# HiKapok/X-Detector

Measured on AMD Instinct MI355X. Metric: images/sec at 480x480 Light-Head R-CNN, 1/2/4/8 MI355X + backbone MFMA util%, higher is better.
Workload: dtype f16x3 (split-precision f16 MFMA, f32 accumulate, f32 activations); 1 GPU; Full Light-Head R-CNN (Xception backbone + RPN + GPU proposals/NMS + PSROIAlign + light head + per-class NMS), 300 proposals, 480x480; batch_per_gpu=256, global_batch=256, image_size=480, concurrent_sub_batches=2, cross_terms=f16, input=whitened f32 [B,3,480,480] resident in HBM, parallelism=image-sharded dp1, weights=seeded random init (no checkpoint exists), graph_replay=True

## Files before the change

include/xdet.h:

```cpp
#ifndef XDET_H_
#define XDET_H_

#include <stddef.h>
#include <stdint.h>

#ifdef __cplusplus
extern "C" {
#endif

#define XDET_OK 0
#define XDET_ERR_INVALID_ARG (-1)
#define XDET_ERR_HIP (-2)
#define XDET_ERR_STATE (-3)
#define XDET_ERR_UNSUPPORTED (-4)

const char* xdet_last_error(void);
int xdet_version(void);
int xdet_device_count(int* n);
int xdet_set_device(int dev);
int xdet_device_pci_bus_id(int dev, char* buf, int buflen);
int xdet_probe_ipc(void);
int xdet_set_default_precision(int mode);
int xdet_get_default_precision(void);

// ... 65 lines not shown
size_t xdet_spectral_conv_workspace_bytes(void* layer, int N);
int xdet_spectral_conv_forward(void* layer, const float* in, int N, int ld_in, void* workspace, float* out, int ld_out,
                               void* stream);
int xdet_stem_conv3x3s2_forward(const float* in_nchw, const float* w27x32, const float* scale, const float* shift,
                                uint16_t* out_hi, uint16_t* out_lo, int N, int S, void* stream);
int xdet_resnet_stem7x7_forward(void* layer, const float* in_nchw, int N, int S, float* out, void* stream);
int xdet_maxpool3x3s2_bn_planes(const float* in, const float* scale, const float* shift, uint16_t* out_hi, uint16_t* out_lo,
                                int N, int H, int W, int C, int ld, float mul, uint16_t* out_hi2, uint16_t* out_lo2,
                                int c32_2, float mul2, void* stream);
int xdet_resnet_preconv_forward(void* layer, const float* pre_scale, const float* pre_shift, const float* x, int N, int H,
                                int W, uint16_t* out_hi, uint16_t* out_lo, void* stream);
int xdet_sepconv_fused_hpool_forward(void* dw_layer, void* pw_layer, const float* in, int N, int H, int W, int ld_in,
                                     float* out_hpooled, int ld_out, int relu_in, void* stream);
int xdet_maxpool_v3s2_add(const float* in_hpooled, const float* residual, float* out, int N, int H, int Wo, int C, int ld,
                          void* stream);
int xdet_maxpool3x3s2_add(const float* in, const float* residual, float* out, int N, int H, int W, int C, int ld,
                          void* stream);
int xdet_nchw_to_nhwc4(const float* in_nchw, float* out_nhwc4, int N, int C, int H, int W, void* stream);
int xdet_preprocess_eval(const uint8_t* image_hwc, int H, int W, float* out_chw, int out_size, void* stream);
enum { XDET_RESIZE_NONE = 1, XDET_RESIZE_CENTRAL_CROP = 2, XDET_RESIZE_PAD_AND_RESIZE = 3, XDET_RESIZE_WARP = 4 };
int xdet_preprocess_eval_batch(const uint8_t* packed, int64_t packed_bytes, const int64_t* offsets,
                               const int32_t* image_shapes, int N, int out_size, int resize, float* out_nchw,
                               float* bbox_img, void* stream);
size_t xdet_preprocess_train_workspace_bytes(int N, int G);
int xdet_preprocess_train_batch(const uint8_t* packed, int64_t packed_bytes, const int64_t* offsets,
                                const int32_t* image_shapes, const int32_t* glabels, const float* gbboxes,
                                const int32_t* n_gt, const int32_t* image_ids , int N, int G,
                                int out_size, uint32_t seed, float* out_nchw, int32_t* out_glabels, float* out_gbboxes,
                                int32_t* out_n_gt, void* records , void* workspace, void* stream);

// ... 173 lines not shown
```

x-detector_amd/csrc/cabi.hip:

```cpp
#include "lighthead.h"
#include "resnet_trunk.h"

namespace xdet {

static thread_local std::string g_last_error;
void set_last_error(const std::string& s) { g_last_error = s; }
int hip_fail(hipError_t e, const char* what, const char* file, int line) {
  char buf[512];
  snprintf(buf, sizeof(buf), "HIP error %d (%s) at %s:%d: %s", (int)e, hipGetErrorString(e), file, line, what);
  g_last_error = buf;
  return XDET_ERR_HIP;
}

static inline hipStream_t S(void* s) { return reinterpret_cast<hipStream_t>(s); }

int g_default_precision = PREC_F32;

}

using namespace xdet;

extern "C" {

const char* xdet_last_error(void) { return g_last_error.c_str(); }
// ... 357 lines not shown
  XDET_REQUIRE(D->ld == ld_in && L->ld_in() == ld_in && L->ld_out() == ld_out && ld_out <= L->cout_pad &&
                   sepconv_fused_supported(ld_in, L->cout_pad, D->dil),
               "sepconv_fused: needs <= 256 input channels (multiple of 32), <= 128 or 129..1024 outputs, dilation 1");
  int Wo, pl;
  same_pad(W, 3, 2, 1, &pl, &Wo);
  DeviceGuard guard(L->device);
  return launch_sepconv_fused(in, D->d_w, L->d_wt_hi_b, L->d_wt_lo_b, L->d_scale, L->d_shift, out_hpooled, N, H, W, ld_in,
                              ld_out, L->cout_pad, relu_in, L->relu_out, S(stream), pl);
}
int xdet_maxpool_v3s2_add(const float* in_hpooled, const float* residual, float* out, int N, int H, int Wo, int C, int ld,
                          void* stream) {
  int Ho, pt;
  same_pad(H, 3, 2, 1, &pt, &Ho);
  return launch_maxpool_v3s2_add(in_hpooled, residual, out, N, H, Wo, C, ld, Ho, pt, S(stream));
}
int xdet_maxpool3x3s2_add(const float* in, const float* residual, float* out, int N, int H, int W, int C, int ld,
                          void* stream) {
  int Ho, Wo, pt, pl;
  same_pad(H, 3, 2, 1, &pt, &Ho);
  same_pad(W, 3, 2, 1, &pl, &Wo);
  return launch_maxpool3x3s2_add(in, residual, out, N, H, W, C, ld, Ho, Wo, pt, pl, S(stream));
}
int xdet_preprocess_eval(const uint8_t* image_hwc, int H, int W, float* out_chw, int out_size, void* stream) {
  return launch_preprocess_eval(image_hwc, H, W, out_chw, out_size, S(stream));
}
int xdet_preprocess_eval_batch(const uint8_t* packed, int64_t packed_bytes, const int64_t* offsets,
                               const int32_t* image_shapes, int N, int out_size, int resize, float* out_nchw,
                               float* bbox_img, void* stream) {
  return launch_preprocess_batch(packed, packed_bytes, offsets, image_shapes, N, out_size, resize, out_nchw, bbox_img,
                                 S(stream));
// ... 101 lines not shown
  XDET_REQUIRE(!n->built, "set_option: the net is already built");
  const std::string k(key), v(value);
  if (k == "large_sep") {
    XDET_REQUIRE(v == "auto" || v == "direct" || v == "spectral", "large_sep must be auto | direct | spectral");
    n->large_sep_mode = v == "auto" ? 0 : v == "direct" ? 1 : 2;
    return XDET_OK;
  }
  if (k == "rpn_stream") {
    XDET_REQUIRE(v == "side" || v == "main", "rpn_stream must be side | main");
    n->rpn_side_stream = v == "side";
    return XDET_OK;
  }
  if (k == "pool_sub") {
    XDET_REQUIRE(v == "on" || v == "off", "pool_sub: on | off");
    n->pool_writes_projection_input = v == "on";
    return XDET_OK;
  }
  if (k == "workspace") {
    XDET_REQUIRE(v == "reuse" || v == "ssa" || v == "poison", "workspace: reuse | ssa | poison");
    XDET_REQUIRE(!(v != "ssa" && n->check_range), "workspace=reuse: check_range validates every tensor after the forward and needs workspace=ssa");
    n->reuse_workspace = v != "ssa";
    n->poison_recycled = v == "poison";
    return XDET_OK;
  }
  if (k == "sepconv") {
    XDET_REQUIRE(v == "fused" || v == "split", "sepconv must be fused | split");
    n->fuse_sepconv = v == "fused";
    return XDET_OK;
  }
  if (k == "ksplit") {
// ... 366 lines not shown
```

x-detector_amd/csrc/common.h:

```cpp
#pragma once
#include <hip/hip_runtime.h>
#include "../../include/xdet.h"
#include "conv_params.h"
#include "workspace.h"
#include <atomic>
#include <cstdint>
#include <cstdio>
#include <string>
#include <vector>

namespace xdet {

void set_last_error(const std::string& s);
int hip_fail(hipError_t e, const char* what, const char* file, int line);

#define XDET_HIP(expr)                                                          \
  do {                                                                          \
    hipError_t _e = (expr);                                                     \
    if (_e != hipSuccess) return ::xdet::hip_fail(_e, #expr, __FILE__, __LINE__); \
  } while (0)

#define XDET_LAUNCH_CHECK() XDET_HIP(hipGetLastError())

#define XDET_REQUIRE(cond, msg)                                   \
// ... 78 lines not shown
                   unsigned short* lo, hipStream_t s);
int launch_dft_inv(const float* Y, int F, int ldn, int C_ld, int N, int m_pad, const float* tab, const float* scale,
                   const float* shift, int relu, float* out, int ldo, int axis, hipStream_t s);

bool sepconv_fused_supported(int cin_ld, int cout_pad, int dil);
int launch_sepconv_fused(const float* in, const float* w9c, const unsigned short* wt_hi_blocked,
                         const unsigned short* wt_lo_blocked, const float* scale, const float* shift, float* out, int N,
                         int H, int W, int ld, int ldo, int cout_pad, int relu_in, int relu_out, hipStream_t s,
                         int pool_pad_l = -1);

bool conv3x3_patch_supported(int kh, int kw, int cin, int cout_pad, int stride, int dil, int pad_mode);
int launch_conv3x3_patch(const unsigned short* in_hi, const unsigned short* in_lo, const unsigned short* wt_hi_blocked,
                         const unsigned short* wt_lo_blocked, const float* scale, const float* shift, float* out, int N, int H,
                         int W, int ldo, int relu, hipStream_t s);

bool resnet_stem7x7_supported(int kh, int kw, int cin, int cout, int stride, int pad_mode, int pad, int S);
int launch_resnet_stem7x7(const float* img_nchw, const unsigned short* wt_hi, const unsigned short* wt_lo, const float* scale,
                          const float* shift, float* out, int N, int S, hipStream_t s);

bool resnet_preconv_supported(int cin, int cmid, int64_t M);
int launch_resnet_preconv(const float* x, const float* pre_sc, const float* pre_sh, const unsigned short* w_hi,
                          const unsigned short* w_lo, const float* sc, const float* sh, unsigned short* out_hi,
                          unsigned short* out_lo, int64_t M, int cin, int cmid, hipStream_t s);

struct BneckLaunch {
  const float* x;
  const float *pre_sc, *pre_sh;
  const unsigned short *wa_hi, *wa_lo, *wb_hi, *wb_lo, *wc_hi, *wc_lo;
  const float *sc_a, *sh_a, *sc_b, *sh_b, *sc_c, *sh_c;
  const float *pl_sc, *pl_sh;
// ... 73 lines not shown
```

x-detector_amd/csrc/lighthead.hip:

```cpp
#include "lighthead.h"

namespace xdet {

static inline double nsplit_of(const ConvLayer* L) { return L->precision == PREC_F16X3 ? 3.0 : 1.0; }

int LightHeadNet::build_body() {
  const float eps = 1e-4f;
  const int S = cfg.image_size;
  in4.H = S; in4.W = S; in4.C = 3;
  XDET_TRY(new_buf(S, S, 3, &in4));
  Buf x, r, t;
  if (g_default_precision != PREC_F32) {
    const HostTensor* kt;
    XDET_TRY(need("block1_conv1/kernel", &kt, {3, 3, 3, 32}));
    std::vector<float> sc, sh;
    float *d_w, *d_sc, *d_sh;
    XDET_TRY(upload(kt->v, &d_w));
    XDET_TRY(upload_bn("block1_conv1_bn", 32, 32, eps, &sc, &sh, &d_sc, &d_sh));
    x = Buf();
    x.H = x.W = (S - 3) / 2 + 1; x.C = 32; x.ld = 32; x.no_f32 = true;
    XDET_TRY(new_planes(&x));
    pscales[x.pidx].name = "block1_conv1 [stem]";
    const Pow2Scaled bn_sc{sc, d_sc}, bn_sh{sh, d_sh};
    pscales[x.pidx].apply.push_back([=](int e) {
// ... 15 lines not shown
  c2.k = 3; c2.cout = 64; c2.pad_mode = 0; c2.relu_out = 1;
  XDET_TRY(conv_bn("block1_conv2", "block1_conv2_bn", eps, ST_BODY, x, c2, &t));
  XDET_REQUIRE(!keep_stem_out || (t.p && !t.no_f32), "plan: stem_out=keep, but block1_conv2 writes no f32 output");
  x = t;
  struct Blk { const char* res; const char* bn; const char* s1; const char* s2; int c; int first_relu; };
  const Blk blks[3] = {{"conv2d_1", "batch_normalization_1", "block2_sepconv1", "block2_sepconv2", 128, 0},
                       {"conv2d_2", "batch_normalization_2", "block3_sepconv1", "block3_sepconv2", 256, 1},
                       {"conv2d_3", "batch_normalization_3", "block4_sepconv1", "block4_sepconv2", 728, 1}};
  Buf presub;
  bool x_is_relu = false;
  for (int bi = 0; bi < 3; ++bi) {
    const Blk& b = blks[bi];
    ConvArgs proj;
    proj.cout = b.c; proj.stride = 2;
    if (presub.hi) proj.presub = &presub;
    XDET_TRY(conv_bn(b.res, b.bn, eps, ST_BODY, x, proj, &r));
    Buf a, p;
    SepArgs s1;
    s1.cout = b.c; s1.pre_relu = x_is_relu ? 0 : b.first_relu; s1.relu_out = 1;
    XDET_TRY(sep_bn(b.s1, eps, ST_BODY, x, s1, &a));
    Buf nsub;
    const bool two_readers = bi < 2 && pool_writes_projection_input && subsample_projections &&
                             g_default_precision != PREC_F32 && b.c % 32 == 0;
    SepArgs s2;
    s2.cout = b.c; s2.pool_res = &r;
    if (two_readers) s2.next_sub = &nsub;
    XDET_TRY(sep_bn(b.s2, eps, ST_BODY, a, s2, &p));
    presub = nsub;
    x_is_relu = nsub.hi != nullptr;
    if (bi == 0 && keep_stem_out) stem_out = x;
    else release_f32(x);
    release_f32(a);
    release_f32(r);
    x = p;
  }
  for (int blk = 5; blk <= 12; ++blk) {
    const Buf res = x;
    Buf a, b2, c3;
    const std::string pre = "block" + std::to_string(blk);
    SepArgs sep;
// ... 325 lines not shown
```

x-detector_amd/csrc/plan.h:

```cpp
#pragma once
#include "layers.h"

#include <array>
#include <functional>
#include <map>
#include <memory>

namespace xdet {

struct HostTensor {
  std::vector<float> v;
  std::vector<int64_t> dims;
};
typedef std::map<std::string, HostTensor> WeightMap;

struct Buf {
  float* p = nullptr;
  unsigned short *hi = nullptr, *lo = nullptr;
  bool planes_relu = false;
  bool no_f32 = false;
  int pidx = -1;
  int H = 0, W = 0, C = 0, ld = 0;
  size_t per_image() const { return (size_t)H * W * ld; }
};

struct ConvEmit {
  int planes = 0;
  const Buf* into = nullptr;
  const std::vector<float>* bn_scale = nullptr;
  const std::vector<float>* bn_shift = nullptr;
  int* optional = nullptr;
  bool ksplit = false;
};

struct ConvArgs {
  int k = 1, cout = 0, stride = 1;
  int pad_mode = 1;
  int pad_expl = 0;
  int relu_out = 0, relu_in = 0;
  const Buf* res = nullptr;
  const float *pre_sc = nullptr, *pre_sh = nullptr;
  const Buf* presub = nullptr;
  ConvEmit emit;
};

struct SepArgs {
  int cout = 0, pre_relu = 0, dilation = 1, relu_out = 0;
  const Buf* res = nullptr;
  const Buf* pool_res = nullptr;
  Buf* next_sub = nullptr;
  ConvEmit emit;
};

struct GraphCache {
  typedef std::array<uintptr_t, 10> Key;
  static constexpr size_t kMax = 8;
  std::map<Key, hipGraphExec_t> execs;
  std::vector<Key> order;
  void clear() {
    for (auto& g : execs) (void)hipGraphExecDestroy(g.second);
    execs.clear();
    order.clear();
  }
  int launch(const Key& key, hipStream_t s, const std::function<int()>& forward) {
    auto it = execs.find(key);
// ... 167 lines not shown

  std::vector<char> planes_drop_ok;
  virtual bool planes_dropped() const { return false; }
  int ksplit_design_batch = 0;
  bool ksplit_all = false;
  static int pow2_floor(int64_t v) { int r = 1; while ((int64_t)r * 2 <= v) r *= 2; return r; }
  int maybe_ksplit(ConvLayer* L, int Hi, int Wi, int Ho, int Wo, bool marked);
  struct KsLayer { ConvLayer* L; bool aux; };
  std::vector<KsLayer> ks_layers;
  float* ks_slab[2] = {nullptr, nullptr};
  int* ks_ticket[2] = {nullptr, nullptr};
  int finish_ksplit();
  bool fuse_sepconv = true;
  bool subsample_projections = true;
  bool pool_writes_projection_input = true;
  bool patch_conv3x3 = true;
  bool fuse_hpool = true;
  int pool_fuse_min_pixels = 100 * 100;
  int add_conv(const std::string& name, int stage, const Buf& in_, ConvLayer* L, const Buf* res, int relu_in, Buf* out,
               const ConvEmit& em = {});
  int add_dw(const std::string& name, int stage, const Buf& in, DepthwiseLayer* L, int relu_in, Buf* out,
             bool planes_only = false);
  int add_pool(const std::string& name, int stage, const Buf& in, const Buf* res, Buf* out);
  ConvLayer* keep(ConvLayer* L) { layers.emplace_back(L); return L; }
  DepthwiseLayer* keep(DepthwiseLayer* L) { layers.emplace_back(L); return L; }
  SpectralConv* keep(SpectralConv* L) { layers.emplace_back(L); return L; }

  int conv_bn(const std::string& name, const std::string& bn, float eps, int stage, const Buf& in, const ConvArgs& args, Buf* out,
              ConvLayer** layer = nullptr);
  int sep_bn(const std::string& name, float eps, int stage, const Buf& in, const SepArgs& args, Buf* out);
// ... 6 lines not shown
```

x-detector_amd/csrc/plan.hip:

```cpp
#include "plan.h"

#include <cstdlib>

namespace xdet {

int Plan::take(size_t bytes, void** out, int kind, size_t slack_bytes) {
  bytes = std::max<size_t>(bytes, 256);
  if (reuse_workspace) {
    auto& fl = ws_free[ws_pool][kind];
    auto it = kind == 1 ? fl.find(bytes) : fl.lower_bound(bytes);
    if (it != fl.end() && it->first <= 2 * bytes) {
      *out = it->second;
      const size_t block = it->first;
      fl.erase(it);
      ws_bytes[*out] = block;
      ws_recycled_bytes += bytes;
      if (poison_recycled && kind == 0 && bytes > slack_bytes)
        poison.push_back({ops.size(), reinterpret_cast<float*>(static_cast<char*>(*out) + (bytes - slack_bytes)),
                          (block - (bytes - slack_bytes)) / 4});
      return XDET_OK;
    }
  }
  XDET_TRY(alloc_bytes(bytes, out));
  ws_bytes[*out] = bytes;
// ... 322 lines not shown
  std::vector<float> sc, sh;
  const float *scp = nullptr, *shp = nullptr;
  if (!bn.empty()) {
    XDET_TRY(fold_bn(bn, cout, eps, nullptr, &sc, &sh));
    scp = sc.data(); shp = sh.data();
  }
  ConvLayer* L = keep(new ConvLayer());
  if (layer) *layer = L;
  XDET_REQUIRE(!pre_sc || (k == 1 && stride == 2 && g_default_precision != PREC_F32 && in.C >= 32 && !in.no_f32 &&
                           in.ld % 32 == 0),
               "plan: a pre-activation can only be folded into a 1x1 stride-2 projection on the split path");
  if (k == 1 && stride == 2 && (pad_mode == 1 || (pad_mode == 2 && pad_expl == 0)) &&
      g_default_precision != PREC_F32 && in.C >= 32 && in.ld % 32 == 0 && !relu_in && !in.no_f32 &&
      (subsample_projections || pre_sc)) {
    XDET_TRY(L->init(1, 1, in.C, cout, 1, 1, 1, 0, 0, kt->v.data(), scp, shp, relu_out));
    if (presub && presub->hi) {
      XDET_REQUIRE(!pre_sc && presub->H == (in.H + 1) / 2 && presub->W == (in.W + 1) / 2 && presub->ld == in.ld,
                   "plan: pre-made subsampled planes do not match the projection's input");
      XDET_TRY(add_conv(name, stage, *presub, L, res, 0, out, emit));
      release_planes(*presub);
      return XDET_OK;
    }
    Buf sub;
    sub.H = (in.H + 1) / 2; sub.W = (in.W + 1) / 2; sub.C = in.C; sub.ld = in.ld; sub.no_f32 = true;
    XDET_TRY(new_planes(&sub));
    pscales[sub.pidx].name = name + "/subsample_split";
    const Buf i = in, o = sub;
    ops.push_back({name + "/subsample_split", stage, 0.0, [=](int N, hipStream_t s) {
                     return launch_split_f32_subsample2(i.p, o.hi, o.lo, N, i.H, i.W, i.ld, s, pre_sc, pre_sh, pmul(o.pidx));
                   }});
    XDET_TRY(add_conv(name, stage, sub, L, res, 0, out, emit));
    release_planes(sub);
    return XDET_OK;
  }
  XDET_REQUIRE(!(presub && presub->hi), "plan: pre-made subsampled planes, but this conv is not a subsampled 1x1 / stride-2 projection");
  XDET_TRY(L->init(k, k, in.C, cout, stride, 1, pad_mode, pad_expl, pad_expl, kt->v.data(), scp, shp, relu_out));
  if (patch_conv3x3 && L->dma_capable() && in.hi && !in.planes_relu && !relu_in && !res && emit.planes == 0 &&
      in.ld == 32 && conv3x3_patch_supported(k, k, in.C, L->cout_pad, stride, 1, pad_mode) && L->cout_pad == L->ld_out()) {
    XDET_TRY(new_buf(in.H - 2, in.W - 2, cout, out));
    if (in.pidx >= 0) pscales[in.pidx].apply.push_back([L](int e) { return L->set_in_exp(e); });
    const Buf i = in, o = *out;
    ops.push_back({name + " [LDS-staged tile]", stage, L->flops(in.H, in.W), [=](int N, hipStream_t s) {
                     return launch_conv3x3_patch(i.hi, i.lo, L->d_wt_hi_b, L->d_wt_lo_b, L->d_scale, L->d_shift, o.p, N, i.H,
                                                 i.W, o.ld, L->relu_out, s);
                   }});
// ... 4 lines not shown

int Plan::sep_bn(const std::string& name, float eps, int stage, const Buf& in, const SepArgs& args, Buf* out) {
  const int cout = args.cout, pre_relu = args.pre_relu, dilation = args.dilation, relu_out = args.relu_out;
  const Buf *res = args.res, *pool_res = args.pool_res;
  Buf* next_sub = args.next_sub;
  const ConvEmit& emit = args.emit;
  const HostTensor *dk, *pk;
  XDET_TRY(need(name + "/depthwise_kernel", &dk, {3, 3, in.C, 1}));
  XDET_TRY(need(name + "/pointwise_kernel", &pk, {1, 1, in.C, cout}));
  DepthwiseLayer* D = keep(new DepthwiseLayer());
  XDET_TRY(D->init(in.C, dilation, dk->v.data()));
  std::vector<float> sc, sh;
  XDET_TRY(fold_bn(name + "_bn", cout, eps, nullptr, &sc, &sh));
  ConvLayer* L = keep(new ConvLayer());
  XDET_TRY(L->init(1, 1, in.C, cout, 1, 1, 1, 0, 0, pk->v.data(), sc.data(), sh.data(), relu_out));
  if (fuse_sepconv && L->dma_capable() && !res && emit.planes == 0 && !in.no_f32 &&
      sepconv_fused_supported(in.ld, L->cout_pad, dilation) && L->ld_out() <= L->cout_pad) {
    {
      PlaneScale ps;
      ps.name = name + " (depthwise result inside the fused block)";
      ps.src = in.p;
      ps.src_per_image = in.per_image();
      ps.src_relu = pre_relu;
      float bound = 0.f;
      for (int c = 0; c < in.C; ++c) {
        float a = 0.f;
        for (int t = 0; t < 9; ++t) a += std::fabs(dk->v[(size_t)t * in.C + c]);
        bound = std::max(bound, a);
      }
      ps.bound = bound;
      ps.apply.push_back([D](int e) { return D->set_out_exp(e); });
      ps.apply.push_back([L](int e) { return L->set_in_exp(e); });
      ps.op_index = (int)ops.size();
      pscales.push_back(ps);
    }
    if (pool_res && fuse_hpool && in.H * in.W >= pool_fuse_min_pixels) {
      int Ho, Wo, pt, pl;
      same_pad(in.H, 3, 2, 1, &pt, &Ho);
      same_pad(in.W, 3, 2, 1, &pl, &Wo);
      Buf hp;
      XDET_TRY(new_buf(in.H, Wo, cout, &hp));
      XDET_TRY(new_buf(Ho, Wo, cout, out));
      XDET_REQUIRE(pool_res->H == Ho && pool_res->W == Wo && pool_res->ld == out->ld && !pool_res->no_f32,
                   "plan: pool residual shape mismatch");
      const Buf i = in, h = hp, o = *out;
      const float* rp = pool_res->p;
      ops.push_back({name + "/fused_dw+pw+hpool", stage, L->flops(in.H, in.W), [=](int N, hipStream_t s) {
                       return launch_sepconv_fused(i.p, D->d_w, L->d_wt_hi_b, L->d_wt_lo_b, L->d_scale, L->d_shift, h.p, N,
                                                   i.H, i.W, i.ld, h.ld, L->cout_pad, pre_relu, L->relu_out, s, pl);
                     }});
      Buf sub;
      if (next_sub && out->ld % 32 == 0) {
        sub.H = (Ho + 1) / 2; sub.W = (Wo + 1) / 2; sub.C = out->C; sub.ld = out->ld; sub.no_f32 = true;
        XDET_TRY(new_planes(&sub));
        pscales[sub.pidx].name = name + "/vpool_add (subsampled planes for the next projection)";
        *next_sub = sub;
      }
      const Buf sb = sub;
      ops.push_back({name + (sb.hi ? "/vpool_add+subsample_split+relu" : "/vpool_add"), stage, 0.0, [=](int N, hipStream_t s) {
                       return launch_maxpool_v3s2_add(h.p, rp, o.p, N, h.H, h.W, h.C, h.ld, Ho, pt, s, sb.hi, sb.lo,
                                                      sb.hi ? pmul(sb.pidx) : 1.f);
                     }});
      release_f32(hp);
      return XDET_OK;
    }
    Buf full;
    Buf* dst = pool_res ? &full : out;
    XDET_TRY(new_buf(in.H, in.W, cout, dst));
    const Buf i = in, o = *dst;
    ops.push_back({name + "/fused_dw+pw", stage, L->flops(in.H, in.W), [=](int N, hipStream_t s) {
                     return launch_sepconv_fused(i.p, D->d_w, L->d_wt_hi_b, L->d_wt_lo_b, L->d_scale, L->d_shift, o.p, N,
                                                 i.H, i.W, i.ld, o.ld, L->cout_pad, pre_relu, L->relu_out, s);
                   }});
    if (!pool_res) return XDET_OK;
    XDET_TRY(add_pool(name + "/pool_add", stage, full, pool_res, out));
    release_f32(full);
    return XDET_OK;
  }
  Buf t, full;
  XDET_TRY(add_dw(name + "/depthwise", stage, in, D, pre_relu, &t, L->dma_capable()));
  XDET_TRY(add_conv(name + "/pointwise", stage, t, L, res, 0, pool_res ? &full : out, emit));
  release_planes(t);
  release_f32(t);
  if (!pool_res) return XDET_OK;
  XDET_TRY(add_pool(name + "/pool_add", stage, full, pool_res, out));
  release_f32(full);
  return XDET_OK;
}

int Plan::run_stage(int stage, int N, hipStream_t s) {
  for (size_t i = 0; i < ops.size(); ++i) {
    const Op& op = ops[i];
    if (op.stage != stage) continue;
    for (const PoisonRec& pr : poison)
      if (pr.op == i) XDET_HIP(hipMemsetD32Async(reinterpret_cast<hipDeviceptr_t>(pr.at), 0x7fc00000, pr.words, s));
    if (profiling) {
      ProfRec r;
      r.op = (int)i;
      XDET_HIP(hipEventCreate(&r.a));
      XDET_HIP(hipEventCreate(&r.b));
      XDET_HIP(hipEventRecord(r.a, s));
// ... 41 lines not shown
```

x-detector_amd/xdet/_lib.py:

```python
import ctypes
import os

_HERE = os.path.dirname(os.path.abspath(__file__))
LIB_PATH = os.environ.get('XDET_LIB') or os.path.join(_HERE, 'libxdet_hip.so')

c_void_p = ctypes.c_void_p
c_int = ctypes.c_int
c_float = ctypes.c_float
c_size_t = ctypes.c_size_t
c_int64 = ctypes.c_int64
c_double = ctypes.c_double
PF = c_void_p
PI = c_void_p


class XdetError(RuntimeError):
    def __init__(self, code, msg):
        RuntimeError.__init__(self, 'xdet error %d: %s' % (code, msg))
        self.code = code


class InvalidArgumentError(XdetError, ValueError):
    """XDET_ERR_INVALID_ARG: the counterpart of tf.errors.InvalidArgumentError raised by the
    reference op's OP_REQUIRES checks (cpp/PSROIPooling/ps_roi_align_op.cc:209-226)."""
# ... 62 lines not shown
    'xdet_sepconv_fused_forward': (c_int, [c_void_p, c_void_p, PF, c_int, c_int, c_int, c_int, PF, c_int, c_int, c_void_p]),
    'xdet_conv3x3_patch_forward': (c_int, [c_void_p, c_void_p, c_void_p, c_int, c_int, c_int, PF, c_int, c_void_p]),
    'xdet_resnet_bneck_forward': (c_int, [c_void_p, c_void_p, c_void_p, PF, PF, PF, c_int, c_int, c_int, PF, PF, PF,
                                          c_void_p, c_void_p, c_void_p]),
    'xdet_spectral_conv_create': (c_int, [ctypes.POINTER(c_void_p), PF, c_int, c_int, c_int, c_int, c_int, PF, PF, c_int]),
    'xdet_spectral_conv_workspace_bytes': (c_size_t, [c_void_p, c_int]),
    'xdet_spectral_conv_forward': (c_int, [c_void_p, PF, c_int, c_int, c_void_p, PF, c_int, c_void_p]),
    'xdet_stem_conv3x3s2_forward': (c_int, [PF, PF, PF, PF, c_void_p, c_void_p, c_int, c_int, c_void_p]),
    'xdet_resnet_stem7x7_forward': (c_int, [c_void_p, PF, c_int, c_int, PF, c_void_p]),
    'xdet_maxpool3x3s2_bn_planes': (c_int, [PF, PF, PF, c_void_p, c_void_p, c_int, c_int, c_int, c_int, c_int, c_float,
                                            c_void_p, c_void_p, c_int, c_float, c_void_p]),
    'xdet_resnet_preconv_forward': (c_int, [c_void_p, PF, PF, PF, c_int, c_int, c_int, c_void_p, c_void_p, c_void_p]),
    'xdet_sepconv_fused_hpool_forward': (c_int, [c_void_p, c_void_p, PF, c_int, c_int, c_int, c_int, PF, c_int, c_int,
                                                 c_void_p]),
    'xdet_maxpool_v3s2_add': (c_int, [PF, PF, PF, c_int, c_int, c_int, c_int, c_int, c_void_p]),
    'xdet_maxpool3x3s2_add': (c_int, [PF, PF, PF, c_int, c_int, c_int, c_int, c_int, c_void_p]),
    'xdet_preprocess_eval': (c_int, [c_void_p, c_int, c_int, PF, c_int, c_void_p]),
    'xdet_preprocess_eval_batch': (c_int, [c_void_p, c_int64, c_void_p, PI, c_int, c_int, c_int, PF, PF, c_void_p]),
    'xdet_preprocess_train_workspace_bytes': (c_size_t, [c_int, c_int]),
    'xdet_preprocess_train_batch': (c_int, [c_void_p, c_int64, c_void_p, PI, PI, PF, PI, PI, c_int, c_int, c_int, ctypes.c_uint32,
                                            PF, PI, PF, PI, c_void_p, c_void_p, c_void_p]),
    'xdet_nchw_to_nhwc4': (c_int, [PF, PF, c_int, c_int, c_int, c_int, c_void_p]),
    'xdet_rpn_decode': (c_int, [PF, c_int, c_int, c_int, c_int, c_int, c_int, c_int, PF, PF, PF, PF, c_void_p]),
    'xdet_proposals_workspace_bytes': (c_size_t, [c_int, c_int, c_int, c_int]),
    'xdet_get_proposals': (c_int, [PF, PF, c_int, c_int, c_int, c_int, c_float, c_float, c_void_p, PF, PI, c_void_p]),
    'xdet_ext_decode_rois': (c_int, [PF, PF, c_int, c_int64, PF, c_void_p]),
    'xdet_bboxes_eval': (c_int, [PF, c_int, PF, c_int, c_int, c_int, PI, PF, c_int, c_int, c_float, c_float, c_int,
                                 PF, PF, c_void_p]),
    'xdet_head_decode_probs': (c_int, [PF, PF, c_int, c_int, c_int, c_int64, c_int, PF, PF, PI, c_void_p]),
    'xdet_bboxes_eval_probs': (c_int, [PF, PF, c_int, c_int, c_int, PI, PF, c_int, c_int, c_float, c_float, c_int, PI,
# ... 130 lines not shown
```

x-detector_amd/xdet/build.py:

```python
import os
import subprocess
import sys

HERE = os.path.dirname(os.path.abspath(__file__))
CSRC = os.path.join(os.path.dirname(HERE), 'csrc')
LIB = os.path.join(HERE, 'libxdet_hip.so')

SOURCES = [
    ('conv_mfma.hip', []),
    ('conv_mfma_split.hip', []),
    ('conv_mfma_dma.hip', []),
    ('conv_mfma_ksplit.hip', []),
    ('elementwise.hip', []),
    ('spectral.hip', []),
    ('sepconv_fused.hip', []),
    ('conv3x3_patch.hip', []),
    ('resnet_bneck.hip', []),
    ('resnet_stem.hip', []),
    ('resnet_preconv.hip', []),
    ('psroialign.hip', ['-ffp-contract=off']),
    ('psroialign_grad_ordered.hip', ['-ffp-contract=off']),
    ('rotated_psroialign.hip', ['-ffp-contract=off']),
    ('proposals.hip', ['-ffp-contract=off']),
    ('detect.hip', ['-ffp-contract=off']),
    ('evalmatch.hip', ['-ffp-contract=off']),
    ('targets.hip', ['-ffp-contract=off']),
    ('losses.hip', ['-ffp-contract=off']),
    ('dense_backward.hip', []),
    ('conv_backward.hip', []),
    ('batchnorm.hip', ['-ffp-contract=off']),
    ('depthwise_backward.hip', ['-ffp-contract=off']),
# ... 48 lines not shown
```

x-detector_amd/xdet/model.py:

```python
import contextlib
import ctypes

import numpy as np

from ._lib import lib, check, c_void_p, LightHeadConfig, XdetError, InvalidArgumentError
from .runtime import DeviceBuffer, DeviceTensor, Stream, to_host, synchronize, _host, _current, _det, _sync
from . import train as _train
from .train import *


class LightHeadDetector(object):
    def __init__(self, weights, image_size=480, max_batch=1, num_classes=21, rpn_pre_nms_top_n=5000,
                 rpn_post_nms_top_n=1000, rpn_nms_thres=0.7, rpn_min_size=None, select_threshold=0.01,
                 nms_threshold=0.3, nms_topk=200, device=None, large_sep='auto', sepconv='fused', rpn_stream='side',
                 conv3x3='patch', pool='split', check_range=False, ksplit=True, cross='f16', workspace=None, pool_sub=None,
                 pool_index=False, rpn_hidden=False, large_sep_train=False, exit_flow_train=False, middle_flow_train=False,
                 entry_flow_train=False):
        stages = (large_sep_train, exit_flow_train, middle_flow_train, entry_flow_train)
        _train.check_stages(stages, weights)
        if device is not None:
            check(lib().xdet_set_device(int(device)))
        self.cfg = LightHeadConfig(image_size=image_size, max_batch=max_batch, num_classes=num_classes,
                                   rpn_pre_nms_top_n=rpn_pre_nms_top_n, rpn_post_nms_top_n=rpn_post_nms_top_n,
                                   rpn_nms_thres=rpn_nms_thres,
                                   rpn_min_size=(16. / 480) if rpn_min_size is None else rpn_min_size,
                                   select_threshold=select_threshold, nms_threshold=nms_threshold, nms_topk=nms_topk)
        h = c_void_p()
        check(lib().xdet_net_create(ctypes.byref(h), ctypes.byref(self.cfg)))
        self.handle = h
        self._head_kernels = {}
        self._rpn_kernels = {}
# ... 3 lines not shown
                self._head_kernels[name] = a
            if rpn_hidden and name in ('rpn_head/conv2d/kernel', 'rpn_head/conv2d_1/kernel', 'rpn_head/conv2d_2/kernel'):
                self._rpn_kernels[name] = a
            dims = (ctypes.c_int64 * a.ndim)(*a.shape)
            check(lib().xdet_net_set_weight(self.handle, name.encode(), _host(a), a.ndim, dims))
        check(lib().xdet_net_set_option(self.handle, b'large_sep', large_sep.encode()))
        check(lib().xdet_net_set_option(self.handle, b'sepconv', sepconv.encode()))
        check(lib().xdet_net_set_option(self.handle, b'rpn_stream', rpn_stream.encode()))
        check(lib().xdet_net_set_option(self.handle, b'conv3x3', conv3x3.encode()))
        check(lib().xdet_net_set_option(self.handle, b'pool', pool.encode()))
        check(lib().xdet_net_set_option(self.handle, b'check_range', b'on' if check_range else b'off'))
        if workspace is not None:
            check(lib().xdet_net_set_option(self.handle, b'workspace', workspace.encode()))
        if pool_sub is not None:
            check(lib().xdet_net_set_option(self.handle, b'pool_sub', pool_sub.encode()))
        check(lib().xdet_net_set_option(self.handle, b'ksplit', ksplit.encode() if isinstance(ksplit, str) else (b'on' if ksplit else b'off')))
        check(lib().xdet_net_set_option(self.handle, b'cross', cross.encode()))
        if pool_index:
            check(lib().xdet_net_set_option(self.handle, b'pool_index', b'keep'))
        if rpn_hidden:
            check(lib().xdet_net_set_option(self.handle, b'rpn_hidden', b'keep'))
        if middle_flow_train:
            check(lib().xdet_net_set_option(self.handle, b'entry_x', b'keep'))
        if entry_flow_train:
            check(lib().xdet_net_set_option(self.handle, b'stem_out', b'keep'))
        self.pool_index, self.rpn_hidden = bool(pool_index), bool(rpn_hidden)
        check(lib().xdet_net_build(self.handle))
        self.max_batch = max_batch
        self.image_size = image_size
        self.num_classes = num_classes
# ... 366 lines not shown
```

x-detector_amd/xdet/ops.py:

```python
import ctypes
import enum

import numpy as np

from ._lib import lib, check, c_void_p, InvalidArgumentError
from .runtime import DeviceBuffer, DeviceTensor, to_device, to_host, synchronize, _ptr, _host, channel_ld


def ps_roi_align(inputs, rois, grid_dim_width, grid_dim_height, pool_method, stream=None):
    if not isinstance(pool_method, str) or ('mean' not in pool_method and 'max' not in pool_method):
        raise InvalidArgumentError(-1, "Need Attr pool_method to be either 'mean' or 'max', got %r" % (pool_method,))
    if grid_dim_width < 0 or grid_dim_height < 0:
        raise InvalidArgumentError(-1, 'Need Attr grid_dim_width/grid_dim_height >= 0')
    inputs = np.asarray(inputs, np.float32)
    rois = np.asarray(rois, np.float32)
    if inputs.ndim != 4:
        raise InvalidArgumentError(-1, "inputs must be in 'NCHW' format.")
    if rois.ndim != 3 or rois.shape[2] != 4:
        raise InvalidArgumentError(-1, "rois must be in 'batch_size x num_rois x 4' format.")
    if inputs.shape[0] != rois.shape[0]:
        raise InvalidArgumentError(-1, "'batch_size' in inputs and rois don't match.")
    N, C, H, W = inputs.shape
    R = rois.shape[1]
    gs = grid_dim_width * grid_dim_height
# ... 303 lines not shown

def separable_block_then_pool_add(op, x, residual, relu_in=False, stream=None):
    N, H, W, C = x.shape
    Ho, Wo = -(-H // 2), -(-W // 2)
    hp = DeviceTensor.empty((N, H, Wo, op.pw.cout))
    out = DeviceTensor.empty((N, Ho, Wo, op.pw.cout))
    st = stream.handle if stream else None
    check(lib().xdet_sepconv_fused_hpool_forward(op.dw.handle, op.pw.handle, x.ptr, N, H, W, x.ld, hp.ptr, hp.ld,
                                                 1 if relu_in else 0, st))
    check(lib().xdet_maxpool_v3s2_add(hp.ptr, residual.ptr if residual is not None else None, out.ptr, N, H, Wo,
                                      op.pw.cout, hp.ld, st))
    synchronize(stream)
    return out


def max_pool_3x3_s2_same_add(x, residual=None, stream=None):
    N, H, W, C = x.shape
    out = DeviceTensor.empty((N, -(-H // 2), -(-W // 2), C))
    check(lib().xdet_maxpool3x3s2_add(x.ptr, residual.ptr if residual is not None else None, out.ptr, N, H, W, C,
                                      x.ld, stream.handle if stream else None))
    return out


def planes_bytes(n_pix, ld):
    return -(-n_pix // 16) * 16 * ld * 2


def _planes_pair(out, n_pix, ld):
    if out is not None:
        return out
# ... 351 lines not shown
```

Measured before the change: 4196 images/sec.

## Fuse residual 1x1 projection into vertical maxpool-add kernel for entry blocks

Defers the strided 1x1 residual projection conv of the first two Xception entry blocks and computes it inside a new kernel that also does the vertical 3x3 max-pool, residual add, subsample split and ReLU. The projection result stays in LDS instead of being written to and reread from HBM as an f32 tensor, and one launch is removed per block. In exchange the projection now runs inside a pool kernel with a 64-pixel tile, which may give lower MFMA efficiency than the dedicated conv kernel and adds LDS pressure (64x256 floats).

```diff
diff --git a/include/xdet.h b/include/xdet.h
--- a/include/xdet.h
+++ b/include/xdet.h
@@ -103,6 +103,9 @@
                                      float* out_hpooled, int ld_out, int relu_in, void* stream);
 int xdet_maxpool_v3s2_add(const float* in_hpooled, const float* residual, float* out, int N, int H, int Wo, int C, int ld,
                           void* stream);
+int xdet_pool_add_projection_forward(void* proj_layer, const float* in_hpooled, const uint16_t* in_hi, const uint16_t* in_lo,
+                                     int N, int H, int Wo, int ld, float* out, uint16_t* sub_hi, uint16_t* sub_lo, int sub_exp,
+                                     void* stream);
 int xdet_maxpool3x3s2_add(const float* in, const float* residual, float* out, int N, int H, int W, int C, int ld,
                           void* stream);
 int xdet_nchw_to_nhwc4(const float* in_nchw, float* out_nhwc4, int N, int C, int H, int W, void* stream);
diff --git a/x-detector_amd/csrc/cabi.hip b/x-detector_amd/csrc/cabi.hip
--- a/x-detector_amd/csrc/cabi.hip
+++ b/x-detector_amd/csrc/cabi.hip
@@ -395,6 +395,22 @@
   same_pad(H, 3, 2, 1, &pt, &Ho);
   return launch_maxpool_v3s2_add(in_hpooled, residual, out, N, H, Wo, C, ld, Ho, pt, S(stream));
 }
+int xdet_pool_add_projection_forward(void* proj_layer, const float* in_hpooled, const uint16_t* in_hi, const uint16_t* in_lo,
+                                     int N, int H, int Wo, int ld, float* out, uint16_t* sub_hi, uint16_t* sub_lo, int sub_exp,
+                                     void* stream) {
+  LayerBase* b = static_cast<LayerBase*>(proj_layer);
+  XDET_REQUIRE(b && b->kind == 1, "not a conv layer");
+  ConvLayer* L = static_cast<ConvLayer*>(b);
+  XDET_REQUIRE(L->dma_capable() && L->groups == 1 && L->kh == 1 && L->kw == 1 && L->stride == 1 && !L->relu_out && L->ksplit < 1 &&
+                   L->ld_out() == ld && pool_add_proj_supported(L->ld_in(), ld, L->cout_pad),
+               "pool_add_projection: needs a 1x1 stride-1 conv without ReLU, 32..256 -> 128 | 256 channels, split-precision mode");
+  XDET_REQUIRE(in_hi && (in_lo || L->precision == PREC_F16) && sub_exp > -64 && sub_exp < 64, "pool_add_projection: bad planes / exponent");
+  int Ho, pt;
+  same_pad(H, 3, 2, 1, &pt, &Ho);
+  DeviceGuard guard(L->device);
+  return launch_pool_add_proj(in_hpooled, in_hi, in_lo, L->d_wt_hi_b, L->d_wt_lo_b, L->d_scale, L->d_shift, out, sub_hi, sub_lo,
+                              ldexpf(1.f, -sub_exp), N, H, Wo, L->ld_in(), ld, L->cout_pad, Ho, pt, S(stream));
+}
 int xdet_maxpool3x3s2_add(const float* in, const float* residual, float* out, int N, int H, int W, int C, int ld,
                           void* stream) {
   int Ho, Wo, pt, pl;
@@ -526,6 +542,11 @@
   if (k == "pool_sub") {
     XDET_REQUIRE(v == "on" || v == "off", "pool_sub: on | off");
     n->pool_writes_projection_input = v == "on";
+    return XDET_OK;
+  }
+  if (k == "pool_proj") {
+    XDET_REQUIRE(v == "fused" || v == "separate", "pool_proj: fused | separate");
+    n->pool_proj_fused = v == "fused";
     return XDET_OK;
   }
   if (k == "workspace") {
diff --git a/x-detector_amd/csrc/common.h b/x-detector_amd/csrc/common.h
--- a/x-detector_amd/csrc/common.h
+++ b/x-detector_amd/csrc/common.h
@@ -116,6 +116,12 @@
                          const unsigned short* wt_lo_blocked, const float* scale, const float* shift, float* out, int N, int H,
                          int W, int ldo, int relu, hipStream_t s);
 
+bool pool_add_proj_supported(int k_ld, int c_ld, int cout_pad);
+int launch_pool_add_proj(const float* in_hpooled, const unsigned short* a_hi, const unsigned short* a_lo,
+                         const unsigned short* wt_hi_blocked, const unsigned short* wt_lo_blocked, const float* scale,
+                         const float* shift, float* out, unsigned short* sub_hi, unsigned short* sub_lo, float sub_mul, int N,
+                         int H, int Wo, int K, int C, int cout_pad, int Ho, int pad_t, hipStream_t s);
+
 bool resnet_stem7x7_supported(int kh, int kw, int cin, int cout, int stride, int pad_mode, int pad, int S);
 int launch_resnet_stem7x7(const float* img_nchw, const unsigned short* wt_hi, const unsigned short* wt_lo, const float* scale,
                           const float* shift, float* out, int N, int S, hipStream_t s);
diff --git a/x-detector_amd/csrc/lighthead.hip b/x-detector_amd/csrc/lighthead.hip
--- a/x-detector_amd/csrc/lighthead.hip
+++ b/x-detector_amd/csrc/lighthead.hip
@@ -53,16 +53,21 @@
     ConvArgs proj;
     proj.cout = b.c; proj.stride = 2;
     if (presub.hi) proj.presub = &presub;
+    const bool two_readers = bi < 2 && pool_writes_projection_input && subsample_projections &&
+                             g_default_precision != PREC_F32 && b.c % 32 == 0;
+    DeferredProj dproj;
+    if (two_readers && pool_proj_fused) proj.defer = &dproj;
+    r = Buf();
     XDET_TRY(conv_bn(b.res, b.bn, eps, ST_BODY, x, proj, &r));
     Buf a, p;
     SepArgs s1;
     s1.cout = b.c; s1.pre_relu = x_is_relu ? 0 : b.first_relu; s1.relu_out = 1;
     XDET_TRY(sep_bn(b.s1, eps, ST_BODY, x, s1, &a));
     Buf nsub;
-    const bool two_readers = bi < 2 && pool_writes_projection_input && subsample_projections &&
-                             g_default_precision != PREC_F32 && b.c % 32 == 0;
     SepArgs s2;
-    s2.cout = b.c; s2.pool_res = &r;
+    s2.cout = b.c;
+    if (dproj.L) s2.pool_proj = &dproj;
+    else s2.pool_res = &r;
     if (two_readers) s2.next_sub = &nsub;
     XDET_TRY(sep_bn(b.s2, eps, ST_BODY, a, s2, &p));
     presub = nsub;
diff --git a/x-detector_amd/csrc/plan.h b/x-detector_amd/csrc/plan.h
--- a/x-detector_amd/csrc/plan.h
+++ b/x-detector_amd/csrc/plan.h
@@ -33,6 +33,12 @@
   bool ksplit = false;
 };
 
+struct DeferredProj {
+  ConvLayer* L = nullptr;
+  std::string name;
+  Buf in;
+};
+
 struct ConvArgs {
   int k = 1, cout = 0, stride = 1;
   int pad_mode = 1;
@@ -41,6 +47,7 @@
   const Buf* res = nullptr;
   const float *pre_sc = nullptr, *pre_sh = nullptr;
   const Buf* presub = nullptr;
+  DeferredProj* defer = nullptr;
   ConvEmit emit;
 };
 
@@ -49,6 +56,7 @@
   const Buf* res = nullptr;
   const Buf* pool_res = nullptr;
   Buf* next_sub = nullptr;
+  const DeferredProj* pool_proj = nullptr;
   ConvEmit emit;
 };
 
@@ -246,6 +254,7 @@
   bool fuse_sepconv = true;
   bool subsample_projections = true;
   bool pool_writes_projection_input = true;
+  bool pool_proj_fused = true;
   bool patch_conv3x3 = true;
   bool fuse_hpool = true;
   int pool_fuse_min_pixels = 100 * 100;
diff --git a/x-detector_amd/csrc/plan.hip b/x-detector_amd/csrc/plan.hip
--- a/x-detector_amd/csrc/plan.hip
+++ b/x-detector_amd/csrc/plan.hip
@@ -360,9 +360,15 @@
       g_default_precision != PREC_F32 && in.C >= 32 && in.ld % 32 == 0 && !relu_in && !in.no_f32 &&
       (subsample_projections || pre_sc)) {
     XDET_TRY(L->init(1, 1, in.C, cout, 1, 1, 1, 0, 0, kt->v.data(), scp, shp, relu_out));
+    const bool defer = args.defer && !res && !relu_out && emit.planes == 0 && L->dma_capable() &&
+                       pool_add_proj_supported(in.ld, L->ld_out(), L->cout_pad);
     if (presub && presub->hi) {
       XDET_REQUIRE(!pre_sc && presub->H == (in.H + 1) / 2 && presub->W == (in.W + 1) / 2 && presub->ld == in.ld,
                    "plan: pre-made subsampled planes do not match the projection's input");
+      if (defer) {
+        *args.defer = {L, name, *presub};
+        return XDET_OK;
+      }
       XDET_TRY(add_conv(name, stage, *presub, L, res, 0, out, emit));
       release_planes(*presub);
       return XDET_OK;
@@ -375,6 +381,10 @@
     ops.push_back({name + "/subsample_split", stage, 0.0, [=](int N, hipStream_t s) {
                      return launch_split_f32_subsample2(i.p, o.hi, o.lo, N, i.H, i.W, i.ld, s, pre_sc, pre_sh, pmul(o.pidx));
                    }});
+    if (defer) {
+      *args.defer = {L, name, sub};
+      return XDET_OK;
+    }
     XDET_TRY(add_conv(name, stage, sub, L, res, 0, out, emit));
     release_planes(sub);
     return XDET_OK;
@@ -409,8 +419,19 @@
   XDET_TRY(fold_bn(name + "_bn", cout, eps, nullptr, &sc, &sh));
   ConvLayer* L = keep(new ConvLayer());
   XDET_TRY(L->init(1, 1, in.C, cout, 1, 1, 1, 0, 0, pk->v.data(), sc.data(), sh.data(), relu_out));
-  if (fuse_sepconv && L->dma_capable() && !res && emit.planes == 0 && !in.no_f32 &&
-      sepconv_fused_supported(in.ld, L->cout_pad, dilation) && L->ld_out() <= L->cout_pad) {
+  const bool fused = fuse_sepconv && L->dma_capable() && !res && emit.planes == 0 && !in.no_f32 &&
+                     sepconv_fused_supported(in.ld, L->cout_pad, dilation) && L->ld_out() <= L->cout_pad;
+  const DeferredProj* pp = args.pool_proj && args.pool_proj->L ? args.pool_proj : nullptr;
+  XDET_REQUIRE(!(pp && pool_res), "plan: a separable block pools against a residual tensor or a deferred projection, not both");
+  const bool fuse_proj = pp && fused && fuse_hpool && in.H * in.W >= pool_fuse_min_pixels && next_sub && L->ld_out() % 32 == 0 &&
+                         pp->L->ld_out() == L->ld_out() && pp->in.hi && pp->in.ld == pp->L->ld_in();
+  Buf proj_res;
+  if (pp && !fuse_proj) {
+    XDET_TRY(add_conv(pp->name, stage, pp->in, pp->L, nullptr, 0, &proj_res));
+    release_planes(pp->in);
+    pool_res = &proj_res;
+  }
+  if (fused) {
     {
       PlaneScale ps;
       ps.name = name + " (depthwise result inside the fused block)";
@@ -429,17 +450,20 @@
       ps.op_index = (int)ops.size();
       pscales.push_back(ps);
     }
-    if (pool_res && fuse_hpool && in.H * in.W >= pool_fuse_min_pixels) {
+    if ((pool_res || fuse_proj) && fuse_hpool && in.H * in.W >= pool_fuse_min_pixels) {
       int Ho, Wo, pt, pl;
       same_pad(in.H, 3, 2, 1, &pt, &Ho);
       same_pad(in.W, 3, 2, 1, &pl, &Wo);
       Buf hp;
       XDET_TRY(new_buf(in.H, Wo, cout, &hp));
       XDET_TRY(new_buf(Ho, Wo, cout, out));
-      XDET_REQUIRE(pool_res->H == Ho && pool_res->W == Wo && pool_res->ld == out->ld && !pool_res->no_f32,
-                   "plan: pool residual shape mismatch");
+      if (fuse_proj)
+        XDET_REQUIRE(pp->in.H == Ho && pp->in.W == Wo && !pp->in.planes_relu, "plan: the deferred projection's planes do not match the pooled map");
+      else
+        XDET_REQUIRE(pool_res->H == Ho && pool_res->W == Wo && pool_res->ld == out->ld && !pool_res->no_f32,
+                     "plan: pool residual shape mismatch");
       const Buf i = in, h = hp, o = *out;
-      const float* rp = pool_res->p;
+      const float* rp = fuse_proj ? nullptr : pool_res->p;
       ops.push_back({name + "/fused_dw+pw+hpool", stage, L->flops(in.H, in.W), [=](int N, hipStream_t s) {
                        return launch_sepconv_fused(i.p, D->d_w, L->d_wt_hi_b, L->d_wt_lo_b, L->d_scale, L->d_shift, h.p, N,
                                                    i.H, i.W, i.ld, h.ld, L->cout_pad, pre_relu, L->relu_out, s, pl);
@@ -452,11 +476,24 @@
         *next_sub = sub;
       }
       const Buf sb = sub;
+      if (fuse_proj) {
+        ConvLayer* P = pp->L;
+        const Buf a = pp->in;
+        if (a.pidx >= 0) pscales[a.pidx].apply.push_back([P](int e) { return P->set_in_exp(e); });
+        ops.push_back({name + "/vpool_add+" + pp->name + "+subsample_split+relu", stage, P->flops(a.H, a.W), [=](int N, hipStream_t s) {
+                         return launch_pool_add_proj(h.p, a.hi, a.lo, P->d_wt_hi_b, P->d_wt_lo_b, P->d_scale, P->d_shift, o.p, sb.hi,
+                                                     sb.lo, pmul(sb.pidx), N, h.H, h.W, a.ld, h.ld, P->cout_pad, Ho, pt, s);
+                       }});
+        release_planes(a);
+        release_f32(hp);
+        return XDET_OK;
+      }
       ops.push_back({name + (sb.hi ? "/vpool_add+subsample_split+relu" : "/vpool_add"), stage, 0.0, [=](int N, hipStream_t s) {
                        return launch_maxpool_v3s2_add(h.p, rp, o.p, N, h.H, h.W, h.C, h.ld, Ho, pt, s, sb.hi, sb.lo,
                                                       sb.hi ? pmul(sb.pidx) : 1.f);
                      }});
       release_f32(hp);
+      release_f32(proj_res);
       return XDET_OK;
     }
     Buf full;
@@ -470,6 +507,7 @@
     if (!pool_res) return XDET_OK;
     XDET_TRY(add_pool(name + "/pool_add", stage, full, pool_res, out));
     release_f32(full);
+    release_f32(proj_res);
     return XDET_OK;
   }
   Buf t, full;
@@ -480,6 +518,7 @@
   if (!pool_res) return XDET_OK;
   XDET_TRY(add_pool(name + "/pool_add", stage, full, pool_res, out));
   release_f32(full);
+  release_f32(proj_res);
   return XDET_OK;
 }
 
diff --git a/x-detector_amd/csrc/pool_add_proj.hip b/x-detector_amd/csrc/pool_add_proj.hip
--- /dev/null
+++ b/x-detector_amd/csrc/pool_add_proj.hip
@@ -0,0 +1,215 @@
+#include "common.h"
+#include "cu_prims.h"
+
+namespace xdet {
+
+struct PoolAddProjParams {
+  const float* in;
+  const u16* a_hi; const u16* a_lo;
+  const u16* wt_hi; const u16* wt_lo;
+  const float* scale; const float* shift;
+  float* out;
+  u16* sub_hi; u16* sub_lo;
+  float sub_mul;
+  int npix, H, Wo, Ho, pad_t, Hs, Ws, nk, cout_pad, ntiles;
+};
+
+__device__ __forceinline__ float4 pap_max4(float4 a, float4 b) {
+  float4 r;
+  asm("v_max_f32 %0, %1, %2" : "=v"(r.x) : "v"(a.x), "v"(b.x));
+  asm("v_max_f32 %0, %1, %2" : "=v"(r.y) : "v"(a.y), "v"(b.y));
+  asm("v_max_f32 %0, %1, %2" : "=v"(r.z) : "v"(a.z), "v"(b.z));
+  asm("v_max_f32 %0, %1, %2" : "=v"(r.w) : "v"(a.w), "v"(b.w));
+  return r;
+}
+
+constexpr int PAP_M = 64;
+
+template <int TN, bool SPLIT3>
+__global__ __launch_bounds__(256, 2) void pool_add_proj_kernel(PoolAddProjParams p) {
+  constexpr int C = 128 * TN, WN = 32 * TN, C4N = C / 4;
+  constexpr int NQ = 4;
+  constexpr int PPQ = 256 / C4N;
+  constexpr int PP = NQ * PPQ;
+  constexpr int NPASS = PAP_M / PP;
+  __shared__ __attribute__((aligned(16))) float s_res[PAP_M * C];
+
+  const int tid = threadIdx.x;
+  const int lane = tid & 63;
+  const int wn = __builtin_amdgcn_readfirstlane(tid >> 6);
+  const int per_xcd = gridDim.x >> 3;
+  const int t = (blockIdx.x & 7) * per_xcd + (blockIdx.x >> 3);
+  if (t >= p.ntiles) return;
+  const int m0 = t * PAP_M;
+
+  const int c = (tid % C4N) * 4, prow = tid / C4N;
+  const int hw = p.Ho * p.Wo;
+  struct Item { int pix, n, oy, ox; bool live; };
+  auto item_of = [&](int pass, int q) {
+    Item it;
+    it.pix = m0 + pass * PP + q * PPQ + prow;
+    it.live = it.pix < p.npix;
+    const int pc = it.live ? it.pix : p.npix - 1;
+    it.n = pc / hw;
+    const int rem = pc - it.n * hw;
+    it.oy = rem / p.Wo;
+    it.ox = rem - it.oy * p.Wo;
+    return it;
+  };
+  auto load_rows = [&](const Item& it, float4 (&rv)[3]) {
+    const float* base = p.in + ((size_t)it.n * p.H * p.Wo + (size_t)it.ox) * C + c;
+    const int iy = it.oy * 2 - p.pad_t;
+#pragma unroll
+    for (int k = 0; k < 3; ++k) {
+      const bool ok = (unsigned)(iy + k) < (unsigned)p.H;
+      rv[k] = *reinterpret_cast<const float4*>(base + (size_t)(ok ? iy + k : 0) * p.Wo * C);
+    }
+  };
+  float4 rows[2][NQ][3];
+#pragma unroll
+  for (int q = 0; q < NQ; ++q) load_rows(item_of(0, q), rows[0][q]);
+  __builtin_amdgcn_sched_barrier(0);
+
+  {
+    const int frow = lane & 31, fh = lane >> 5;
+    f32x16 acc[2][TN];
+#pragma unroll
+    for (int i = 0; i < 2; ++i)
+#pragma unroll
+      for (int j = 0; j < TN; ++j)
+#pragma unroll
+        for (int r = 0; r < 16; ++r) acc[i][j][r] = 0.f;
+    size_t aoff[2];
+    bool aok[2];
+#pragma unroll
+    for (int i = 0; i < 2; ++i) {
+      const int pix = m0 + i * 32 + frow;
+      aok[i] = pix < p.npix;
+      aoff[i] = (((size_t)(pix >> 4) * p.nk) << 9) + (size_t)(((pix & 15) << 5) + fh * 8);
+    }
+    const f16x8 zero = {0, 0, 0, 0, 0, 0, 0, 0};
+#pragma unroll 1
+    for (int kt = 0; kt < p.nk; ++kt) {
+      f16x8 ah[2][2], al[2][2], bh[TN][2], bl[TN][2];
+#pragma unroll
+      for (int i = 0; i < 2; ++i)
+#pragma unroll
+        for (int ks = 0; ks < 2; ++ks) {
+          const size_t o = aoff[i] + ((size_t)kt << 9) + ks * 16;
+          ah[i][ks] = aok[i] ? *reinterpret_cast<const f16x8*>(p.a_hi + o) : zero;
+          if (SPLIT3) al[i][ks] = aok[i] ? *reinterpret_cast<const f16x8*>(p.a_lo + o) : zero;
+        }
+#pragma unroll
+      for (int j = 0; j < TN; ++j)
+#pragma unroll
+        for (int ks = 0; ks < 2; ++ks) {
+          const size_t o = ((size_t)kt * p.cout_pad + (wn * WN + j * 32 + frow)) * 32 + (ks * 2 + fh) * 8;
+          bh[j][ks] = *reinterpret_cast<const f16x8*>(p.wt_hi + o);
+          if (SPLIT3) bl[j][ks] = *reinterpret_cast<const f16x8*>(p.wt_lo + o);
+        }
+#pragma unroll
+      for (int ks = 0; ks < 2; ++ks) {
+        if (SPLIT3) {
+#pragma unroll
+          for (int i = 0; i < 2; ++i)
+#pragma unroll
+            for (int j = 0; j < TN; ++j) acc[i][j] = __builtin_amdgcn_mfma_f32_32x32x16_f16(al[i][ks], bh[j][ks], acc[i][j], 0, 0, 0);
+#pragma unroll
+          for (int i = 0; i < 2; ++i)
+#pragma unroll
+            for (int j = 0; j < TN; ++j) acc[i][j] = __builtin_amdgcn_mfma_f32_32x32x16_f16(ah[i][ks], bl[j][ks], acc[i][j], 0, 0, 0);
+        }
+#pragma unroll
+        for (int i = 0; i < 2; ++i)
+#pragma unroll
+          for (int j = 0; j < TN; ++j) acc[i][j] = __builtin_amdgcn_mfma_f32_32x32x16_f16(ah[i][ks], bh[j][ks], acc[i][j], 0, 0, 0);
+      }
+    }
+#pragma unroll
+    for (int j = 0; j < TN; ++j) {
+      const int co = wn * WN + j * 32 + frow;
+      const float esc = p.scale[co], esh = p.shift[co];
+#pragma unroll
+      for (int i = 0; i < 2; ++i)
+#pragma unroll
+        for (int r = 0; r < 16; ++r)
+          s_res[(i * 32 + (r & 3) + 8 * (r >> 2) + 4 * fh) * C + co] = fmaf(acc[i][j][r], esc, esh);
+    }
+  }
+  __syncthreads();
+
+#pragma unroll
+  for (int pass = 0; pass < NPASS; ++pass) {
+    if (pass + 1 < NPASS) {
+#pragma unroll
+      for (int q = 0; q < NQ; ++q) load_rows(item_of(pass + 1, q), rows[(pass + 1) & 1][q]);
+    }
+#pragma unroll
+    for (int q = 0; q < NQ; ++q) {
+      const Item it = item_of(pass, q);
+      const int iy = it.oy * 2 - p.pad_t;
+      float4 rv[3];
+#pragma unroll
+      for (int k = 0; k < 3; ++k) {
+        const bool ok = (unsigned)(iy + k) < (unsigned)p.H;
+        float4 v = rows[pass & 1][q][k];
+        v.x = ok ? v.x : -INFINITY; v.y = ok ? v.y : -INFINITY; v.z = ok ? v.z : -INFINITY; v.w = ok ? v.w : -INFINITY;
+        rv[k] = v;
+      }
+      float4 m = pap_max4(pap_max4(rv[0], rv[1]), rv[2]);
+      const float4 r = *reinterpret_cast<const float4*>(&s_res[(pass * PP + q * PPQ + prow) * C + c]);
+      m.x += r.x; m.y += r.y; m.z += r.z; m.w += r.w;
+      if (!it.live) continue;
+      if (!((it.oy | it.ox) & 1)) {
+        const int64_t pix = ((int64_t)it.n * p.Hs + (it.oy >> 1)) * p.Ws + (it.ox >> 1);
+        const size_t po = ((size_t)((pix >> 4) * (C >> 5) + (c >> 5)) << 9) + ((size_t)(pix & 15) << 5) + (size_t)(c & 31);
+        const float v[4] = {m.x * p.sub_mul, m.y * p.sub_mul, m.z * p.sub_mul, m.w * p.sub_mul};
+        _Float16 h[4], l[4];
+#pragma unroll
+        for (int k = 0; k < 4; ++k) {
+          h[k] = (_Float16)v[k];
+          l[k] = (_Float16)(v[k] - (float)h[k]);
+        }
+        *reinterpret_cast<uint2*>(p.sub_hi + po) = *reinterpret_cast<const uint2*>(h);
+        *reinterpret_cast<uint2*>(p.sub_lo + po) = *reinterpret_cast<const uint2*>(l);
+      }
+      m.x = !(m.x <= 0.f) ? m.x : 0.f; m.y = !(m.y <= 0.f) ? m.y : 0.f; m.z = !(m.z <= 0.f) ? m.z : 0.f; m.w = !(m.w <= 0.f) ? m.w : 0.f;
+      *reinterpret_cast<float4*>(p.out + (size_t)it.pix * C + c) = m;
+    }
+  }
+}
+
+bool pool_add_proj_supported(int k_ld, int c_ld, int cout_pad) {
+  return k_ld % 32 == 0 && k_ld >= 32 && k_ld <= 256 && (c_ld == 128 || c_ld == 256) && cout_pad == c_ld;
+}
+
+int launch_pool_add_proj(const float* in_hpooled, const unsigned short* a_hi, const unsigned short* a_lo,
+                         const unsigned short* wt_hi_blocked, const unsigned short* wt_lo_blocked, const float* scale,
+                         const float* shift, float* out, unsigned short* sub_hi, unsigned short* sub_lo, float sub_mul, int N,
+                         int H, int Wo, int K, int C, int cout_pad, int Ho, int pad_t, hipStream_t s) {
+  XDET_REQUIRE(pool_add_proj_supported(K, C, cout_pad), "pool_add_proj: needs 32..256 input channels (multiple of 32) and 128 | 256 outputs");
+  XDET_REQUIRE(in_hpooled && a_hi && (a_lo || !wt_lo_blocked) && wt_hi_blocked && scale && shift && out && sub_hi && sub_lo,
+               "pool_add_proj: NULL argument");
+  XDET_REQUIRE(N >= 0 && H > 0 && Wo > 0 && Ho > 0 && pad_t >= 0 && 2 * (Ho - 1) - pad_t < H, "pool_add_proj: bad geometry");
+  const int64_t npix = (int64_t)N * Ho * Wo;
+  if (npix == 0) return XDET_OK;
+  XDET_REQUIRE(npix + PAP_M < ((int64_t)1 << 31), "pool_add_proj: too many output pixels for one launch");
+  PoolAddProjParams p;
+  p.in = in_hpooled; p.a_hi = a_hi; p.a_lo = a_lo; p.wt_hi = wt_hi_blocked; p.wt_lo = wt_lo_blocked; p.scale = scale; p.shift = shift;
+  p.out = out; p.sub_hi = sub_hi; p.sub_lo = sub_lo; p.sub_mul = sub_mul;
+  p.npix = (int)npix; p.H = H; p.Wo = Wo; p.Ho = Ho; p.pad_t = pad_t; p.Hs = (Ho + 1) / 2; p.Ws = (Wo + 1) / 2;
+  p.nk = K / 32; p.cout_pad = cout_pad; p.ntiles = (int)cdiv(npix, PAP_M);
+  const dim3 grid((unsigned)(cdiv(p.ntiles, 8) * 8));
+  const bool split3 = wt_lo_blocked != nullptr;
+  if (C == 128) {
+    if (split3) hipLaunchKernelGGL((pool_add_proj_kernel<1, true>), grid, dim3(256), 0, s, p);
+    else hipLaunchKernelGGL((pool_add_proj_kernel<1, false>), grid, dim3(256), 0, s, p);
+  } else {
+    if (split3) hipLaunchKernelGGL((pool_add_proj_kernel<2, true>), grid, dim3(256), 0, s, p);
+    else hipLaunchKernelGGL((pool_add_proj_kernel<2, false>), grid, dim3(256), 0, s, p);
+  }
+  XDET_LAUNCH_CHECK();
+  return XDET_OK;
+}
+
+}
diff --git a/x-detector_amd/xdet/_lib.py b/x-detector_amd/xdet/_lib.py
--- a/x-detector_amd/xdet/_lib.py
+++ b/x-detector_amd/xdet/_lib.py
@@ -100,6 +100,8 @@
     'xdet_sepconv_fused_hpool_forward': (c_int, [c_void_p, c_void_p, PF, c_int, c_int, c_int, c_int, PF, c_int, c_int,
                                                  c_void_p]),
     'xdet_maxpool_v3s2_add': (c_int, [PF, PF, PF, c_int, c_int, c_int, c_int, c_int, c_void_p]),
+    'xdet_pool_add_projection_forward': (c_int, [c_void_p, PF, c_void_p, c_void_p, c_int, c_int, c_int, c_int, PF, c_void_p,
+                                                 c_void_p, c_int, c_void_p]),
     'xdet_maxpool3x3s2_add': (c_int, [PF, PF, PF, c_int, c_int, c_int, c_int, c_int, c_void_p]),
     'xdet_preprocess_eval': (c_int, [c_void_p, c_int, c_int, PF, c_int, c_void_p]),
     'xdet_preprocess_eval_batch': (c_int, [c_void_p, c_int64, c_void_p, PI, c_int, c_int, c_int, PF, PF, c_void_p]),
diff --git a/x-detector_amd/xdet/build.py b/x-detector_amd/xdet/build.py
--- a/x-detector_amd/xdet/build.py
+++ b/x-detector_amd/xdet/build.py
@@ -15,6 +15,7 @@
     ('spectral.hip', []),
     ('sepconv_fused.hip', []),
     ('conv3x3_patch.hip', []),
+    ('pool_add_proj.hip', []),
     ('resnet_bneck.hip', []),
     ('resnet_stem.hip', []),
     ('resnet_preconv.hip', []),
diff --git a/x-detector_amd/xdet/model.py b/x-detector_amd/xdet/model.py
--- a/x-detector_amd/xdet/model.py
+++ b/x-detector_amd/xdet/model.py
@@ -14,7 +14,7 @@
                  rpn_post_nms_top_n=1000, rpn_nms_thres=0.7, rpn_min_size=None, select_threshold=0.01,
                  nms_threshold=0.3, nms_topk=200, device=None, large_sep='auto', sepconv='fused', rpn_stream='side',
                  conv3x3='patch', pool='split', check_range=False, ksplit=True, cross='f16', workspace=None, pool_sub=None,
-                 pool_index=False, rpn_hidden=False, large_sep_train=False, exit_flow_train=False, middle_flow_train=False,
+                 pool_proj=None, pool_index=False, rpn_hidden=False, large_sep_train=False, exit_flow_train=False, middle_flow_train=False,
                  entry_flow_train=False):
         stages = (large_sep_train, exit_flow_train, middle_flow_train, entry_flow_train)
         _train.check_stages(stages, weights)
@@ -48,6 +48,8 @@
             check(lib().xdet_net_set_option(self.handle, b'workspace', workspace.encode()))
         if pool_sub is not None:
             check(lib().xdet_net_set_option(self.handle, b'pool_sub', pool_sub.encode()))
+        if pool_proj is not None:
+            check(lib().xdet_net_set_option(self.handle, b'pool_proj', pool_proj.encode()))
         check(lib().xdet_net_set_option(self.handle, b'ksplit', ksplit.encode() if isinstance(ksplit, str) else (b'on' if ksplit else b'off')))
         check(lib().xdet_net_set_option(self.handle, b'cross', cross.encode()))
         if pool_index:
diff --git a/x-detector_amd/xdet/ops.py b/x-detector_amd/xdet/ops.py
--- a/x-detector_amd/xdet/ops.py
+++ b/x-detector_amd/xdet/ops.py
@@ -341,6 +341,16 @@
     return out
 
 
+def pool_add_projection(proj, hp, in_planes, out, sub_planes, sub_exp=0, stream=None):
+    N, H, Wo, C = hp.shape
+    assert C == proj.cout and out.shape == (N, -(-H // 2), Wo, C) and out.ld == hp.ld, (hp.shape, out.shape, proj.cout)
+    check(lib().xdet_pool_add_projection_forward(proj.handle, hp.ptr, in_planes[0].ptr, in_planes[1].ptr, N, H, Wo, hp.ld, out.ptr,
+                                                 sub_planes[0].ptr, sub_planes[1].ptr, int(sub_exp),
+                                                 stream.handle if stream else None))
+    synchronize(stream)
+    return out
+
+
 def max_pool_3x3_s2_same_add(x, residual=None, stream=None):
     N, H, W, C = x.shape
     out = DeviceTensor.empty((N, -(-H // 2), -(-W // 2), C))
```

Measured after the change: 4231 images/sec (median of 6 runs). No clear change (+0.8%).
